# THU-luvision/TextureFusion

Measured on AMD Instinct MI355X. Metric: RGB-D frames/s (TSDF integrate + atlas update: prepare->integrate->finalize, UpdateMeshes, GeneratePatches + UpdateAtlas over the frame's dirty chunks), higher is better.
Workload: dtype f32

## Files before the change

### texturefusion_amd/csrc/tf_mesh.hip

```cpp
#include <stdlib.h>
#include <string.h>

#include <algorithm>
#include <vector>

#include "tf_devfn.h"
#include "tf_kf_store.h"
#include "tf_mc_table.h"
#include "tf_patch_body.h"
#include "tf_volume.h"

#pragma clang fp contract(off)

namespace tf {

__device__ const unsigned long long d_mc_tri[256] = TF_MC_TRI_TABLE_INIT;

constexpr int kR = 11;
constexpr int kRS = 11;
constexpr int kPS = kRS * kR;
constexpr int kRV = kPS * kR;
constexpr int kEdgeSlots = 3 * 729;
__device__ __forceinline__ uint32_t mesh_shard_rows_d(uint32_t max_chunks) { return max_chunks / kMeshShards + 258u; }

// ... 293 lines not shown
template <bool WAVE_FORM, bool PATCH, bool TL = false>
__global__ __launch_bounds__(256, PATCH ? (WAVE_FORM ? TF_FILTER_PATCH_WAVES : TF_FILTER_BATCH_WAVES) : (WAVE_FORM ? TF_FILTER_WAVES : TF_FILTER_BATCH_WAVES)) void k_mesh_filter(VolumeDev v, const int4* __restrict__ dlist,
                                                     const uint32_t* __restrict__ dslot,
                                                     const uint32_t* __restrict__ dcount, uint32_t max_entries,
                                                     uint32_t epoch, uint32_t* __restrict__ surv,
                                                     uint32_t* __restrict__ cnt, uint32_t cap_sh, int ppar, bool use_summ,
                                                     uint32_t* __restrict__ len_hint, int shards_par, FilterPatch fp) {
  if (fp.n_store && blockIdx.x == 0) {
    kf_store_body<256>(v, fp.store.tab, fp.store.slots, fp.store.arena, fp.store.cap, fp.store.slot, fp.store.slack, fp.store.fill);
    return;
  }
  const uint32_t bx = blockIdx.x - fp.n_store, nbx = gridDim.x - fp.n_store;
  if (PATCH && bx - fp.first < fp.n_patch) {
    patch_body<true, true, true>(v, fp.cam, fp.par, fp.kf, bx - fp.first, fp.n_patch);
    return;
  }
  const uint32_t bid = PATCH ? (fp.first ? bx : bx - fp.n_patch) : bx;
  const uint32_t nblk = PATCH ? nbx - fp.n_patch : nbx;
  const int lane = threadIdx.x & 63, w = threadIdx.x >> 6;
  const bool is_near = lane < 27 && (lane % 3) >= 1 && ((lane / 3) % 3) >= 1 && lane / 9 >= 1;
  const uint32_t create_seq = v.vctl->create_seq;
  const uint32_t tl_wave = (bid * 256 + threadIdx.x) >> 6;
  bool tl_first = true;
  auto stamp = [&](int k, bool wait) {
    if (TL && tl_first && tl_wave < (uint32_t)kPhaseWaves) {
      if (wait) asm volatile("s_waitcnt vmcnt(0)" ::: "memory");
      if (lane == 0) v.phase_buf[tl_wave * 16 + k] = __builtin_amdgcn_s_memrealtime();
    }
  };
  if (TL && lane == 0 && tl_wave < (uint32_t)kPhaseWaves) { for (int k = 1; k < 8; ++k) v.phase_buf[tl_wave * 16 + k] = 0; }
  stamp(0, false);
  uint32_t n_flat = *dcount;
  if (n_flat > max_entries) n_flat = max_entries;
  const uint32_t wl_rows = mesh_shard_rows_d(v.max_chunks);
  const size_t wl_base = (size_t)(shards_par & 1) * kMeshShards * wl_rows;
  uint32_t sh_n = 0, sh_incl = 0;
  if (shards_par >= 0 && (!WAVE_FORM || bid == 0)) {
    if (lane < (int)kMeshShards) { sh_n = v.wl_cnt[((shards_par & 1) * kMeshShards + lane) * 16]; if (sh_n > wl_rows) sh_n = wl_rows; }
    sh_incl = sh_n;
#pragma unroll
    for (int o = 1; o < (int)kMeshShards; o <<= 1) {
      const uint32_t u = (uint32_t)__shfl_up((int)sh_incl, o);
      if (lane >= o) sh_incl += u;
    }
  }
  const uint32_t n_sh = (uint32_t)__builtin_amdgcn_readfirstlane(__shfl((int)sh_incl, kMeshShards - 1));
  uint32_t n = n_flat + n_sh;
  if (n > max_entries) n = max_entries;
  if (len_hint && bid == 0 && threadIdx.x == 0) *len_hint = n;
  const uint32_t nwaves = nblk * 4;
  if (WAVE_FORM) {
    const uint32_t wave = (uint32_t)__builtin_amdgcn_readfirstlane((int)((bid * 256 + threadIdx.x) >> 6));
    auto process = [&](const int4 id, const uint32_t own_listed, const bool have_own) {
      if (fp.cls && ((fp.cls == 1u) != part_interior(v, id.x, id.y, id.z))) return;
      const uint32_t own = have_own ? own_listed : hash_slot_alive(v, pack_id(id.x, id.y, id.z));
      if (own == kInvalidSlot) return;
      const bool claimed = have_own && id.w > 0;
      const uint32_t roww = load_here(&v.nbr[(size_t)own * kNbrWords + (lane & (kNbrWords - 1))]);
      const uint32_t alivew = v.hent[claimed ? (uint32_t)id.w - 1u : 0u].alive;
      uint32_t w = lane < kNbrWords ? roww : 0u;
      const uint32_t alive = claimed ? (alivew & 1u) : 1u;
      stamp(2, true);
      if (!alive) return;
      w = nbr_row_checked(v, own, id, lane, w, create_seq);
      const uint32_t nslot = lane == 13 ? own : ((lane < 27 && w) ? w - 1u : kInvalidSlot);
      if (use_summ) {
        const uint32_t sm = (is_near && nslot != kInvalidSlot) ? v.summ[nslot] : 0u;
        const uint32_t sel = lane == 13 ? 0u : ((lane % 3) == 2 ? 4u : (((lane / 3) % 3) == 2 ? 8u : 12u));
        const uint32_t u = is_near ? (sm >> sel) & 15u : 0u;
        const bool so = (__shfl((int)sm, 13) & 1) != 0;
        stamp(3, true);
        const bool maybe = so && __ballot(u & 2u) != 0ull && __ballot(u & 4u) != 0ull && __ballot(u & 8u) != 0ull;
        if (!maybe) {
          if (lane == 0) { if (fp.defer) filter_defer_reset(v, cnt, cap_sh, own, id); else filter_reset_record(v, own, id, epoch, ppar); }
          stamp(4, true);
          return;
        }
      }
      filter_exact<true>(v, id, nslot, own, lane, epoch, surv, cnt, cap_sh, ppar, use_summ, fp.defer != 0, create_seq);
      stamp(5, true);
    };
    if (shards_par >= 0) {
      const uint32_t sd = wave & (kMeshShards - 1u);
      const uint32_t stride = (nwaves - sd + kMeshShards - 1u) / kMeshShards;
      uint32_t i = wave / kMeshShards;
      size_t at = wl_base + (size_t)sd * wl_rows + (i < wl_rows ? i : 0u);
      const unsigned long long* const idq = reinterpret_cast<const unsigned long long*>(&v.wl_ids[at]);
      const unsigned long long id_lo = load_here(idq), id_hi = load_here(idq + 1);
      uint32_t own_listed = load_here(&v.wl_slot[at]);
      uint32_t cs = load_here(&v.wl_cnt[((shards_par & 1) * kMeshShards + sd) * 16]);
      int4 id = make_int4((int)(uint32_t)id_lo, (int)(uint32_t)(id_lo >> 32), (int)(uint32_t)id_hi, (int)(uint32_t)(id_hi >> 32));
      if (cs > wl_rows) cs = wl_rows;
      stamp(1, true);
      while (i < cs) {
        process(id, own_listed, true);
        stamp(6, false);
        tl_first = false;
        i += stride;
        if (i < cs) { at = wl_base + (size_t)sd * wl_rows + i; id = v.wl_ids[at]; own_listed = v.wl_slot[at]; }
      }
    }
    for (uint32_t entry = wave; entry < n_flat; entry += nwaves) {
      const int4 id = dlist[entry];
      uint32_t own_listed = kInvalidSlot;
      if (dslot) own_listed = dslot[entry];
      process(id, own_listed, dslot != nullptr);
    }
    return;
  }
  __shared__ uint32_t s_n, s_ne;
  __shared__ uint32_t s_incl[kMeshShards], s_cnt[kMeshShards];
  if (threadIdx.x < kMeshShards) { s_incl[threadIdx.x] = sh_incl; s_cnt[threadIdx.x] = sh_n; }
  __shared__ uint32_t s_eown[32];
  __shared__ int4 s_eid[32];
  __shared__ int4 s_id[32];
  __shared__ uint32_t s_own[32];
  const int grp = threadIdx.x >> 3, k8 = threadIdx.x & 7;
  const uint32_t per = (n + nblk - 1) / nblk;
  const uint32_t first = bid * per;
  const uint32_t last = first + per < n ? first + per : n;
  for (uint32_t base = first; base < last; base += 32u) {
    if (threadIdx.x == 0) { s_n = 0; s_ne = 0; }
    __syncthreads();
    const uint32_t entry = base + (uint32_t)grp;
    if (entry < last) {
      int4 id;
      uint32_t own_in = kInvalidSlot;
      if (entry < n_flat) {
        id = dlist[entry];
        own_in = dslot ? dslot[entry] : hash_slot_alive(v, pack_id(id.x, id.y, id.z));
      } else {
        const uint32_t r = entry - n_flat;
        uint32_t shd = 0;
        for (uint32_t q = 0; q < kMeshShards; ++q) shd += s_incl[q] <= r ? 1u : 0u;
        shd &= kMeshShards - 1u;
        const size_t at = wl_base + (size_t)shd * wl_rows + (r - (s_incl[shd] - s_cnt[shd]));
        id = v.wl_ids[at];
        own_in = v.wl_slot[at];
      }
      uint32_t own;
      bool maybe;
      filter_near(v, id, lane, k8, own_in, dslot != nullptr || entry >= n_flat, use_summ, create_seq, &own, &maybe);
      if (fp.cls && ((fp.cls == 1u) != part_interior(v, id.x, id.y, id.z))) own = kInvalidSlot;
      if (own != kInvalidSlot && k8 == 0) {
        if (maybe) {
          const uint32_t at = atomicAdd(&s_n, 1u);
          s_own[at] = own; s_id[at] = id;
        } else {
          const uint32_t at = atomicAdd(&s_ne, 1u);
          s_eown[at] = own; s_eid[at] = id;
        }
      }
    }
    __syncthreads();
    if (w == 3 && lane < (int)s_ne) {
      if (fp.defer) filter_defer_reset(v, cnt, cap_sh, s_eown[lane], s_eid[lane]);
      else filter_reset_record(v, s_eown[lane], s_eid[lane], epoch, ppar);
    }
    const uint32_t nm = s_n;
    for (uint32_t m = (uint32_t)w; m < nm; m += 4u)
      filter_exact<false>(v, s_id[m], kInvalidSlot, s_own[m], lane, epoch, surv, cnt, cap_sh, ppar, use_summ, fp.defer != 0, create_seq);
    __syncthreads();
  }
}

__device__ __forceinline__ void mesh_stamp(const VolumeDev& v, uint32_t r, int k) {
  if (threadIdx.x == 0 && blockIdx.x < (uint32_t)kPhaseWaves && r == blockIdx.x)
    v.phase_buf[blockIdx.x * 16 + k] = __builtin_amdgcn_s_memrealtime();
}

#ifndef TF_MESH_WAVES
#define TF_MESH_WAVES 6
#endif
template <int NT, bool DBG = false>
__global__ __launch_bounds__(NT, TF_MESH_WAVES) void k_mesh(VolumeDev v, const uint32_t* __restrict__ surv, uint32_t* __restrict__ cnt,
                                                 uint32_t* __restrict__ cnt_next, uint32_t cap_sh,
                                                 uint32_t epoch, float res, uint32_t simplified, uint32_t dbg,
                                                 int rearm) {
  __shared__ MeshSh<NT> sh;
  extern __shared__ uint16_t vlist[];
  const int t = threadIdx.x, lane = t & 63;
  uint32_t n_rows = 0, excl_l = 0, incl_l = 0;
  {
    uint32_t my_n = cnt[(lane & 31) * 16 + (lane >> 5)];
    if (my_n > cap_sh) my_n = cap_sh;
    uint32_t incl = my_n;
#pragma unroll
    for (int o = 1; o < 64; o <<= 1) {
      const uint32_t u = (uint32_t)__shfl_up((int)incl, o);
      if (lane >= o) incl += u;
    }
    n_rows = (uint32_t)__builtin_amdgcn_readfirstlane(__shfl((int)incl, 63));
    const uint32_t r0 = blockIdx.x;
    const uint32_t sh0 = (uint32_t)__popcll(__ballot(incl <= r0));
    incl_l = (uint32_t)__builtin_amdgcn_readfirstlane(__shfl((int)incl, (int)(sh0 & 63u)));
    excl_l = incl_l - (uint32_t)__builtin_amdgcn_readfirstlane(__shfl((int)my_n, (int)(sh0 & 63u)));
    incl_l = (uint32_t)__builtin_amdgcn_readfirstlane((int)sh0);
  }
  if (blockIdx.x == 0 && t < (int)kMeshShards) { cnt_next[t * 16] = 0u; cnt_next[t * 16 + 1] = 0u; cnt_next[(kMeshShards + t) * 16] = 0u; cnt_next[(kMeshShards + t) * 16 + 1] = 0u; cnt_next[(2 * kMeshShards + t) * 16] = 0u; }
  if (blockIdx.x < kMeshShards) {
    uint32_t n_reset = cnt[(2u * kMeshShards + blockIdx.x) * 16u];
    if (n_reset > cap_sh) n_reset = cap_sh;
    for (uint32_t i = (uint32_t)t; i < n_reset; i += NT) {
      const int4 e = v.reset_list[(size_t)blockIdx.x * cap_sh + i];
      filter_reset_record(v, (uint32_t)e.w, make_int4(e.x, e.y, e.z, 0), epoch, rearm >= 0 ? (rearm ^ 1) : -1);
    }
  }
  const float half = res * 0.5f;
  if (rearm >= 0 && blockIdx.x == 0 && t == 0) {
    AtlasCtl::Set* O = &v.actl->set[rearm];
    O->n_work = 0; O->n_cand = 0; O->n_patch = 0; O->slots_base = 0ull;
    v.actl->set[rearm ^ 1].slots_base = v.actl->n_slots;
  }
  if (rearm >= 0 && blockIdx.x == 0 && t < (int)kMeshShards) {
    v.patch_cnt[((rearm & 1) * kMeshShards + t) * 16] = 0u;
    v.wl_cnt[((rearm & 1) * kMeshShards + t) * 16] = 0u;
  }
  if (DBG && dbg == 9) mesh_stamp(v, blockIdx.x, 0);
  for (uint32_t r = blockIdx.x; r < n_rows; r += gridDim.x) {
    uint32_t shard, own;
    int4 id;
    float2 a[512 / NT];
    unsigned long long htab[(kHalo + NT - 1) / NT];
    uint32_t rstate0, rblock0, rpress0;
    unsigned long long rtexloc0;
    {
      shard = incl_l;
      uint32_t idx = r - excl_l;
      if (r != blockIdx.x) {
        uint32_t my_n = cnt[(lane & 31) * 16 + (lane >> 5)];
        if (my_n > cap_sh) my_n = cap_sh;
        uint32_t incl = my_n;
#pragma unroll
        for (int o = 1; o < 64; o <<= 1) {
          const uint32_t u = (uint32_t)__shfl_up((int)incl, o);
          if (lane >= o) incl += u;
        }
        shard = (uint32_t)__builtin_amdgcn_readfirstlane((int)__popcll(__ballot(incl <= r)));
        idx = r - (uint32_t)__builtin_amdgcn_readfirstlane(__shfl((int)incl, (int)(shard & 63u)) - __shfl((int)my_n, (int)(shard & 63u)));
      }
      if (shard >= kMeshShards) { shard -= kMeshShards; idx = cap_sh - 1u - idx; }
      const size_t row = (size_t)shard * cap_sh + idx;
      own = surv[32 * row + 13];
      id = make_int4((int)surv[32 * row + 27], (int)surv[32 * row + 28], (int)surv[32 * row + 29], 0);
#pragma unroll
      for (int j = 0; j < 512 / NT; ++j) a[j] = v.tsdf[(size_t)own * kChunkVoxels + j * NT + t];
      const uint32_t roww = load_here(&surv[32 * row + (t & 31)]);
      int th = threadIdx.x;
      asm volatile("" : "+v"(th));
#pragma unroll
      for (int j = 0; j < (kHalo + NT - 1) / NT; ++j) {
        const int at = j * NT + th;
        const unsigned long long e = d_mesh_tabs.halo[(j + 1) * NT <= kHalo ? at : (at < kHalo ? at : kHalo - 1)];
        htab[j] = ((j + 1) * NT <= kHalo || at < kHalo) ? e : ~0ull;
      }
      const MeshRec* const rec0 = &v.mesh_rec[own];
      rstate0 = rec0->state; rblock0 = rec0->block; rpress0 = blk_pressure(v); rtexloc0 = rec0->texloc;
      __syncthreads();
      if (t < 27) sh.nslot[t] = roww;
    }
    int t_ = threadIdx.x;
    asm volatile("" : "+v"(t_));
    const int t = t_, lane = t & 63, w = t >> 6;
    MeshRec* rec = &v.mesh_rec[own];
    if (DBG && dbg == 9) mesh_stamp(v, r, 1);
    if (t == 0) { sh.nv = 0; sh.nt = 0; sh.adj = 0; sh.ncell = 0; }
    if (DBG && dbg == 1) continue;
#pragma unroll
    for (int j = 0; j < 512 / NT; ++j) {
      const int q = j * NT + t;
      const int x0 = q & 7, y0 = (q >> 3) & 7, z0 = q >> 6;
      sh.S[ridx(x0, y0, z0)] = a[j].x; sh.cflag[x0 + y0 * 9 + z0 * 81] = (a[j].y > 50.0f) ? kCfHeavy : 0u;
    }
    if (t == NT - 64) { sh.rstate = rstate0; sh.rblock = rblock0; sh.rtexloc = rtexloc0; sh.rpress = rpress0; }
    __syncthreads();
    float4 hv[(kHalo + NT - 1) / NT];
    bool hhave[(kHalo + NT - 1) / NT];
#pragma unroll
    for (int j = 0; j < (kHalo + NT - 1) / NT; ++j) {
      const unsigned long long e = htab[j];
      const uint32_t nb = (uint32_t)(e >> 11) & 31u;
      const uint32_t s = sh.nslot[nb < 26u ? nb : 26u];
      hhave[j] = e != ~0ull && s != kInvalidSlot;
      hv[j] = reinterpret_cast<const float4*>(v.tsdf + (size_t)(hhave[j] ? s : own) * kChunkVoxels)[hhave[j] ? (uint32_t)(e >> 16) & 255u : 0u];
    }
#pragma unroll
    for (int j = 0; j < (kHalo + NT - 1) / NT; ++j) {
      const unsigned long long e = htab[j];
      const float4 val = hhave[j] ? hv[j] : make_float4(999.0f, 0.0f, 999.0f, 0.0f);
      const uint32_t r0 = (uint32_t)e & 2047u;
      if (e != ~0ull && ((e >> 24) & 1ull)) {
        sh.S[r0] = val.x;
        const uint32_t cf = (uint32_t)(e >> 26) & 1023u;
        if (cf) sh.cflag[cf - 1u] = (val.y > 50.0f) ? kCfHeavy : 0u;
      }
      if (e != ~0ull && ((e >> 25) & 1ull)) {
        sh.S[r0 + 1u] = val.z;
        const uint32_t cf = (uint32_t)(e >> 36) & 1023u;
        if (cf) sh.cflag[cf - 1u] = (val.w > 50.0f) ? kCfHeavy : 0u;
      }
    }
    __syncthreads();
    if (DBG && dbg == 9) mesh_stamp(v, r, 3);
    for (int c = t; c < 729; c += NT) {
      const int r = ridx(c % 9, (c / 9) % 9, c / 81);
      const float xm = sh.S[r - 1], xp = sh.S[r + 1], ym = sh.S[r - kRS], yp = sh.S[r + kRS];
      const float zm = sh.S[r - kPS], zp = sh.S[r + kPS];
      uint32_t f = (xm < 1.0f ? 1u : 0u) | (xp < 1.0f ? 2u : 0u) | (ym < 1.0f ? 4u : 0u) | (yp < 1.0f ? 8u : 0u) |
                   (zm < 1.0f ? 16u : 0u) | (zp < 1.0f ? 32u : 0u);
      const float gx = xp - xm, gy = yp - ym, gz = zp - zm;
      const float yz = gy * gy + gz * gz;
      const float nrm = sqrtf(gx * gx + yz);
      if (!(nrm > res * 100.0f)) f |= kCfGradOk;
      sh.cflag[c] |= (uint8_t)f;
    }
    for (int i = t; i < (kEdgeSlots + 7) / 8; i += NT) sh.ownq[i] = 0u;
    __syncthreads();

    if (DBG && dbg == 2) continue;
    if (DBG && dbg == 9) mesh_stamp(v, r, 4);
    for (int cell = t; cell < 512; cell += NT) {
      const int x = cell & 7, y = (cell >> 3) & 7, z = cell >> 6;
      const int c0 = ridx(x, y, z);
      bool observed = true;
      int pos = 0, index = 0;
#pragma unroll
      for (int k = 0; k < 8; ++k) {
        const float s = sh.S[c0 + cox(k) + coy(k) * kRS + coz(k) * kPS];
        observed = observed && !(s > 1.0f);
        pos += (s > 0.0f) ? 1 : 0;
        index |= (0.0f > s) ? (1 << k) : 0;
      }
      sh.cinfo[cell] = 0;
      if (observed && (pos % 8) > 0 && index != 0 && index != 255)
        sh.clist[atomicAdd(&sh.ncell, 1u)] = (uint16_t)cell;
    }
    __syncthreads();
    if (t == 0 && sh.ncell) atomicAdd(&cnt[(kMeshShards + shard) * 16 + 1], 1u);
    for (uint32_t ci = t; ci < sh.ncell; ci += NT) {
      const int cell = sh.clist[ci];
      const int x = cell & 7, y = (cell >> 3) & 7, z = cell >> 6;
      const int c0 = ridx(x, y, z);
      float cube[8];
      int index = 0;
#pragma unroll
      for (int k = 0; k < 8; ++k) {
        const float s = sh.S[c0 + cox(k) + coy(k) * kRS + coz(k) * kPS];
        cube[k] = s;
        index |= (0.0f > s) ? (1 << k) : 0;
      }
      const unsigned long long row = d_mc_tri[index];
      uint32_t valid = 0;
      const int cf0 = x + y * 9 + z * 81;
#pragma unroll
      for (int e = 0; e < 12; ++e) {
        const int e0 = (int)((0x321076543210ull >> (4 * e)) & 0xF), e1 = (int)((0x765447650321ull >> (4 * e)) & 0xF);
        const float s0 = cube[e0], s1 = cube[e1];
        const bool far = fabsf(s0) > fabsf(s1);
        const int ko = far ? (cox(e1) + coy(e1) * 9 + coz(e1) * 81) : (cox(e0) + coy(e0) * 9 + coz(e0) * 81);
        const uint32_t need0 = kCfHeavy | kCfGradOk | (1u << cox(e0)) | (4u << coy(e0)) | (16u << coz(e0));
        const uint32_t need1 = kCfHeavy | kCfGradOk | (1u << cox(e1)) | (4u << coy(e1)) | (16u << coz(e1));
        const uint32_t need = far ? need1 : need0;
        if (s0 * s1 < 0.0f) {
          const uint32_t have = sh.cflag[cf0 + ko];
          if ((have & need) == need) valid |= 1u << e;
        }
      }
      uint32_t ntri = 0, used = 0;
#pragma unroll 1
      for (int col = 0; col < 15; col += 3) {
        const int s0 = (int)((row >> (4 * col)) & 0xF);
        if (s0 == 0xF) break;
        const int s1 = (int)((row >> (4 * col + 4)) & 0xF), s2 = (int)((row >> (4 * col + 8)) & 0xF);
        if (!((valid >> s0) & (valid >> s1) & (valid >> s2) & 1u)) continue;
        ++ntri;
        used |= (1u << s0) | (1u << s1) | (1u << s2);
      }
      for (uint32_t u = used; u; u &= u - 1) {
        const int e = __builtin_ctz(u);
        const int m = edge_slot(x, y, z, e);
        atomicOr(&sh.ownq[m >> 3], 1u << (4 * (m & 7) + edge_q(e)));
      }
      sh.cinfo[cell] = (uint16_t)(used | (ntri << 12));
      sh.cidx[cell] = (uint8_t)index;
    }
    __syncthreads();

    if (DBG && dbg == 3) continue;
    if (DBG && dbg == 9) mesh_stamp(v, r, 5);
    {
      constexpr int kEpt = 2304 / NT, kCpt = 512 / NT;
      const int first = t * kEpt;
      unsigned long long usedm = 0;
      {
        constexpr int kWords = (kEpt * 4 + 31) / 32 + 1;
        const int w0 = first >> 3, sh0 = 4 * (first & 7);
#pragma unroll
        for (int q = 0; q < kWords; ++q) {
          const int wi = w0 + q;
          uint32_t x = wi < (kEdgeSlots + 7) / 8 ? sh.ownq[wi] : 0u;
          x |= x >> 1; x |= x >> 2; x &= 0x11111111u;
          x = (x | (x >> 3)) & 0x03030303u;
          x = (x | (x >> 6)) & 0x000F000Fu;
          x = (x | (x >> 12)) & 0xFFu;
          usedm |= (unsigned long long)x << (8 * q);
        }
        usedm >>= (sh0 >> 2);
        usedm &= (1ull << kEpt) - 1ull;
        const int left = kEdgeSlots - first;
        if (left < kEpt) usedm = left > 0 ? (usedm & ((1ull << left) - 1ull)) : 0ull;
      }
      const uint32_t cnt = (uint32_t)__popcll(usedm);
      uint32_t tc = 0;
#pragma unroll
      for (int j = 0; j < kCpt; ++j) tc += (uint32_t)sh.cinfo[kCpt * t + j] >> 12;
      uint32_t pk = cnt | (tc << 16);
      uint32_t inc = pk;
#pragma unroll
      for (int o = 1; o < 64; o <<= 1) {
        const uint32_t u = __shfl_up(inc, o);
        if (lane >= o) inc += u;
      }
      if (lane == 63) sh.wsum[w] = inc;
      __syncthreads();
      uint32_t before = 0, total = 0;
      for (int k = 0; k < NT / 64; ++k) {
        if (k < w) before += sh.wsum[k];
        total += sh.wsum[k];
      }
      if (t == 0) sh.ovf = mesh_block_for(v, sh.rblock, total & 0xFFFFu, total >> 16, sh.rpress);
      __syncthreads();
      const uint32_t ovf_blk = sh.ovf;
      uint16_t* const gvl = (ovf_blk != kBlkFail && (ovf_blk & kBlkLarge)) ? v.ovf_vlist + (size_t)((ovf_blk & ~kBlkLarge) - 1u) * kOvfCV : nullptr;
      const uint32_t excl = before + inc - pk;
      uint32_t r = excl & 0xFFFFu;
      sh.rbase[t] = (uint16_t)r;
      sh.rmask[t] = usedm;
      for (unsigned long long u = usedm; u; u &= u - 1ull) {
        const int m = first + (int)__builtin_ctzll(u);
        if (gvl) { if (r < (uint32_t)kOvfCV) gvl[r] = (uint16_t)m; }
        else if (r < v.mesh_cv) vlist[r] = (uint16_t)m;
        ++r;
      }
      uint32_t t0 = excl >> 16;
#pragma unroll
      for (int j = 0; j < kCpt; ++j) {
        sh.toff[kCpt * t + j] = (uint16_t)t0;
        t0 += (uint32_t)sh.cinfo[kCpt * t + j] >> 12;
      }
      if (t == 0) { sh.nv = total & 0xFFFFu; sh.nt = total >> 16; }
    }
    __syncthreads();
    const uint32_t nv = sh.nv, nt = sh.nt;
    const uint32_t ovf = sh.ovf;
    if (ovf == kBlkFail) {
      if (t == 0) {
        atomicOr(&v.vctl->status, kStMeshFull);
        const uint32_t was = sh.rstate & kMsInMap;
        rec->nv = 0; rec->nt = 0; rec->state = was | kMsOverflow; rec->epoch = epoch;
        if (rearm >= 0 && was) patch_list_append(v, rearm ^ 1, shard, id, own, sh.rtexloc, sh.rblock);
      }
      __syncthreads();
      continue;
    }
    const uint16_t* const gvlist = (ovf & kBlkLarge) ? v.ovf_vlist + (size_t)((ovf & ~kBlkLarge) - 1u) * kOvfCV : nullptr;

    if (DBG && dbg == 4) continue;
    if (DBG && dbg == 9) mesh_stamp(v, r, 6);
    const uint32_t inmap = (sh.rstate & kMsInMap) | (nv ? kMsInMap : 0u);
    if (t == NT - 64) {
      mesh_block_settle(v, sh.rblock, ovf);
      if (rearm >= 0 && inmap) patch_list_append(v, rearm ^ 1, shard, id, own, sh.rtexloc, ovf);
    }
    const float org[3] = {(float)(8 * id.x) * res, (float)(8 * id.y) * res, (float)(8 * id.z) * res};
    uint32_t adj = 0;
    for (uint32_t i = t; i < nv; i += NT) {
      const int m = gvlist ? gvlist[i] : vlist[i];
      const int cell = owner_cell(m, __builtin_ctz((sh.ownq[m >> 3] >> (4 * (m & 7))) & 0xFu));
      const int x = cell & 7, y = (cell >> 3) & 7, z = cell >> 6;
      const int ax = m % 3, b = m / 3;
      const int bx = b % 9, by = (b / 9) % 9, bz = b / 81;
      const int e = edge_of_slot(ax, bx - x, by - y, bz - z);
      const int e0 = edge_c0(e), e1 = edge_c1(e);
      const float s0 = sh.S[ridx(x + cox(e0), y + coy(e0), z + coz(e0))];
      const float s1 = sh.S[ridx(x + cox(e1), y + coy(e1), z + coz(e1))];
      const float tt = s0 / (s0 - s1);
      const int o0[3] = {cox(e0), coy(e0), coz(e0)}, o1[3] = {cox(e1), coy(e1), coz(e1)};
      const int cc[3] = {x, y, z};
      float pv[3];
#pragma unroll
      for (int a = 0; a < 3; ++a) {
        const float p0 = (float)o0[a] * res, p1 = (float)o1[a] * res;
        const float ev = p0 + tt * (p1 - p0);
        const float origin = org[a] + ((float)cc[a] * res + half);
        pv[a] = ev + origin;
      }
      const int k = (fabsf(s0) > fabsf(s1)) ? e1 : e0;
      const int px = x + cox(k), py = y + coy(k), pz = z + coz(k);
      float g[3];
      gradient_at(sh.S, px, py, pz, cox(k), coy(k), coz(k), res, g);
      const uint32_t cs = sh.nslot[((px + 8) >> 3) + ((py + 8) >> 3) * 3 + ((pz + 8) >> 3) * 9];
      const unsigned long long c4 = load_here(reinterpret_cast<const unsigned long long*>(v.color + (size_t)cs * kChunkVoxels + (px & 7) + (py & 7) * 8 + (pz & 7) * 64));
      float col[3] = {1.0f, 1.0f, 1.0f};
      const float cw = (float)(uint16_t)(c4 >> 48);
      if (cw > 0.0f) {
        col[0] = ((float)(uint16_t)c4 / 255.0f) / cw;
        col[1] = ((float)(uint16_t)(c4 >> 16) / 255.0f) / cw;
        col[2] = ((float)(uint16_t)(c4 >> 32) / 255.0f) / cw;
      }
#pragma unroll
      for (int a = 0; a < 3; ++a) {
        mesh_plane(v, ovf, kMpPos + a)[i] = pv[a];
        mesh_plane(v, ovf, kMpNrm + a)[i] = g[a];
        mesh_plane(v, ovf, kMpCol + a)[i] = col[a];
        const int gp = (int)floorf((pv[a] - org[a]) / (res * 1.0f));
        if (gp >= 8) adj |= 1u << (2 * a + 1);
        if (gp <= 0) adj |= 1u << (2 * a);
      }
    }
    if (adj) atomicOr(&sh.adj, adj);
    if (DBG && dbg == 9) mesh_stamp(v, r, 7);
    for (uint32_t ci = (uint32_t)(NT - 1 - t); ci < sh.ncell; ci += NT) {
      const int cell = sh.clist[ci];
      const uint32_t info = sh.cinfo[cell];
      if (!(info >> 12)) continue;
      const int x = cell & 7, y = (cell >> 3) & 7, z = cell >> 6;
      const unsigned long long row = d_mc_tri[sh.cidx[cell]];
      const uint32_t valid = info & 0xFFFu;
      uint32_t o = sh.toff[cell];
      for (int col = 0; col < 15; col += 3) {
        const int s0 = (int)((row >> (4 * col)) & 0xF);
        if (s0 == 0xF) break;
        const int s1 = (int)((row >> (4 * col + 4)) & 0xF), s2 = (int)((row >> (4 * col + 8)) & 0xF);
        if (!((valid >> s0) & (valid >> s1) & (valid >> s2) & 1u)) continue;
        constexpr int kEptT = 2304 / NT;
        auto ref_of = [&](int m) {
          const int tt = m / kEptT, j = m - tt * kEptT;
          return (uint16_t)(sh.rbase[tt] + (uint32_t)__popcll(sh.rmask[tt] & ((1ull << j) - 1ull)));
        };
        tri_plane(v, ovf, 0)[o] = ref_of(edge_slot(x, y, z, s2));
        tri_plane(v, ovf, 1)[o] = ref_of(edge_slot(x, y, z, s1));
        tri_plane(v, ovf, 2)[o] = ref_of(edge_slot(x, y, z, s0));
        ++o;
      }
    }
    __syncthreads();
    if (t == 0) {
      rec->nv = (uint16_t)nv; rec->nt = (uint16_t)nt; rec->epoch = epoch; rec->block = ovf;
      rec->state = inmap | (sh.adj << kMsAdjShift) | (inmap ? simplified : 0u);
    }
    __syncthreads();
    if (DBG && dbg == 9) mesh_stamp(v, r, 8);
  }
}

__global__ __launch_bounds__(256) void k_init_mesh_rec(MeshRec* rec, uint32_t n) {
  for (uint32_t i = blockIdx.x * 256 + threadIdx.x; i < n; i += gridDim.x * 256) {
    MeshRec r;
    memset(&r, 0, sizeof(r));
    r.texloc = kNoTexloc;
    r.frameid = -1;
    r.ratio[0] = r.ratio[1] = 1.0f;
    rec[i] = r;
  }
}
void launch_init_meshes(const VolumeDev& v, hipStream_t s) {
  hipLaunchKernelGGL(k_init_mesh_rec, dim3(1024), dim3(256), 0, s, v.mesh_rec, v.max_chunks);
  (void)hipMemsetAsync(v.mesh_rec + v.max_chunks, 0, sizeof(uint32_t) * ((size_t)blk_ring_len(v.mesh_blocks) + blk_ring_len(v.ovf_blocks)), s);
  (void)hipMemsetAsync(v.mesh_cnt, 0, sizeof(uint32_t) * 2 * kMeshCntWords, s);
}

uint32_t mesh_shard_rows(uint32_t max_chunks) { return max_chunks / kMeshShards + 258u; }

static void launch_mesher(const VolumeDev& v, int cnt_par, uint32_t max_entries, uint32_t epoch, float res, bool fused,
                          int rearm_set, hipStream_t s) {
  static const uint32_t dbg = getenv("TF_MESH_DBG") ? (uint32_t)atoi(getenv("TF_MESH_DBG")) : 0u;
  uint32_t* surv = v.mesh_nbr;
  uint32_t* cnt = v.mesh_cnt + (size_t)(cnt_par & 1) * kMeshCntWords;
  uint32_t* cnt_next = v.mesh_cnt + (size_t)((cnt_par & 1) ^ 1) * kMeshCntWords;
  const uint32_t cap_sh = mesh_shard_rows(v.max_chunks);
  uint32_t grid = ((max_entries + kMeshShards - 1) / kMeshShards + 1) * kMeshShards;
  static const uint32_t gmax = (uint32_t)device_cus() * (uint32_t)(TF_MESH_WAVES * 2);
  if (grid > gmax) grid = gmax;
  if (dbg)
    hipLaunchKernelGGL((k_mesh<128, true>), dim3(grid), dim3(128), v.mesh_cv * sizeof(uint16_t), s, v, surv, cnt, cnt_next, cap_sh, epoch, res,
                       fused ? kMsSimplified : 0u, dbg, rearm_set);
  else
    hipLaunchKernelGGL((k_mesh<128>), dim3(grid), dim3(128), v.mesh_cv * sizeof(uint16_t), s, v, surv, cnt, cnt_next, cap_sh, epoch, res,
                       fused ? kMsSimplified : 0u, 0u, rearm_set);
}

bool launch_mesh(const VolumeDev& v, int cnt_par, const int4* dlist, const uint32_t* dcount, uint32_t max_entries,
                 uint32_t epoch, float res, bool fused, int rearm_set, uint32_t len_guess, uint32_t* len_hint, int shards_par,
                 hipStream_t s, const PatchStage* patch, const Cam* cam, int cls, const KfStoreArgs* store) {
  if (!max_entries) return false;
  uint32_t* cnt = v.mesh_cnt + (size_t)(cnt_par & 1) * kMeshCntWords;
  const uint32_t cap_sh = mesh_shard_rows(v.max_chunks);
  if (max_entries > v.max_chunks) max_entries = v.max_chunks;
  const uint32_t fmax = 2560u;
  const uint32_t fgrid = (max_entries + 3) / 4 < fmax ? (max_entries + 3) / 4 : fmax;
  const uint32_t* dslot = fused ? v.work_slot : nullptr;
  const int ppar = fused ? (rearm_set ^ 1) : -1;
  const bool use_summ = true;
  const bool wave_form = len_guess <= 2560u * 4u;
  FilterPatch fp;
  memset(&fp, 0, sizeof(fp));
  fp.cls = (uint32_t)cls;
  if (store) { fp.n_store = 1u; fp.store = *store; }
  if (patch && cam) {
    fp.defer = 1u;
    fp.n_patch = 1024u;
    fp.first = 0u;
    fp.par = patch->par;
    fp.cam = *cam;
    fp.kf = patch->kf;
  }
#define TF_LAUNCH_FILTER(W, P)                                                                                       \
  hipLaunchKernelGGL((k_mesh_filter<W, P>), dim3(fgrid + fp.n_patch + fp.n_store), dim3(256), 0, s, v, dlist, dslot, dcount, max_entries, \
                     epoch, v.mesh_nbr, cnt, cap_sh, ppar, use_summ, len_hint, shards_par, fp)
  static const bool tl = getenv("TF_MESH_DBG") && atoi(getenv("TF_MESH_DBG")) == 10;
  if (wave_form && tl && !fp.n_patch)
    hipLaunchKernelGGL((k_mesh_filter<true, false, true>), dim3(fgrid + fp.n_store), dim3(256), 0, s, v, dlist, dslot, dcount, max_entries,
                       epoch, v.mesh_nbr, cnt, cap_sh, ppar, use_summ, len_hint, shards_par, fp);
  else if (wave_form) { if (fp.n_patch) TF_LAUNCH_FILTER(true, true); else TF_LAUNCH_FILTER(true, false); }
  else { if (fp.n_patch) TF_LAUNCH_FILTER(false, true); else TF_LAUNCH_FILTER(false, false); }
#undef TF_LAUNCH_FILTER
  launch_mesher(v, cnt_par, max_entries, epoch, res, fused, rearm_set, s);
  return fp.n_patch != 0;
}

constexpr uint32_t kDirtyBlocks = 512;
__device__ __forceinline__ void dirty_frame_body(const VolumeDev& v, int par, uint32_t stamp) {
  const SelBuf& L = v.sel;
  const uint32_t nl = L.ctl->n_list <= v.max_list ? L.ctl->n_list : 0u;
  const uint32_t total = nl * 8u;
  AtlasCtl::Set* S = &v.actl->set[par];
  const int lane = threadIdx.x & 63, w = threadIdx.x >> 6;
  __shared__ uint32_t wcnt[16];
  __shared__ uint32_t gbase;
  for (uint32_t b0 = blockIdx.x * 1024; b0 < total; b0 += kDirtyBlocks * 1024) {
    const uint32_t t = b0 + threadIdx.x;
    bool emit = false;
    int4 q = make_int4(0, 0, 0, 0);
    uint32_t slot = kInvalidSlot;
    if (t < total && (t & 7u) != 7u) {
      const uint32_t e = list_phys(v, t >> 3, L.ctl->n_front);
      const int k = (int)(t & 7u);
      const int4 id0 = L.list_id[e];
      const uint32_t slot0 = L.list_slot[e];
      if (L.list_needs[e]) {
        q = nbr7(id0, k);
        q.w = 0;
        if (k == 0) slot = slot0;
        else slot = hash_slot_alive(v, pack_id(q.x, q.y, q.z));
        if (slot != kInvalidSlot && part_owned(v, q.x, q.y, q.z))
          emit = atomicMax(&v.mesh_rec[slot].stamp, stamp) < stamp;
      }
    }
    const unsigned long long m = __ballot(emit);
    if (lane == 0) wcnt[w] = (uint32_t)__popcll(m);
    __syncthreads();
    if (threadIdx.x == 0) {
      uint32_t tot = 0;
      for (int k = 0; k < 16; ++k) { const uint32_t c = wcnt[k]; wcnt[k] = tot; tot += c; }
      gbase = tot ? atomicAdd(&S->n_work, tot) : 0u;
    }
    __syncthreads();
    if (emit) {
      const uint32_t p = gbase + wcnt[w] + (uint32_t)__popcll(m & ((1ull << lane) - 1ull));
// ... 438 lines not shown
```

Before: 11070.

## Fuse corner-flag pass into cell classification and compute flags lazily per active cell

Drops the separate pass that computed neighbour-observed and gradient-ok flags for all 729 corners. Those flags are now computed on demand only for the corners of surface-crossing cells. Cell classification is restructured so each thread walks a z-column and reuses the previous z-plane's four samples, which roughly halves the shared-memory reads, and one __syncthreads is removed. The trade-off is redundant flag work for corners shared by several active cells, plus more register pressure and divergence inside the active-cell loop.

New measurement: 11140, median of 3. Within noise of the previous version (+0.6%).

```diff
diff --git a/texturefusion_amd/csrc/tf_mesh.hip b/texturefusion_amd/csrc/tf_mesh.hip
--- a/texturefusion_amd/csrc/tf_mesh.hip
+++ b/texturefusion_amd/csrc/tf_mesh.hip
@@ -619,40 +619,37 @@
     }
     __syncthreads();
     if (DBG && dbg == 9) mesh_stamp(v, r, 3);
-    for (int c = t; c < 729; c += NT) {
-      const int r = ridx(c % 9, (c / 9) % 9, c / 81);
-      const float xm = sh.S[r - 1], xp = sh.S[r + 1], ym = sh.S[r - kRS], yp = sh.S[r + kRS];
-      const float zm = sh.S[r - kPS], zp = sh.S[r + kPS];
-      uint32_t f = (xm < 1.0f ? 1u : 0u) | (xp < 1.0f ? 2u : 0u) | (ym < 1.0f ? 4u : 0u) | (yp < 1.0f ? 8u : 0u) |
-                   (zm < 1.0f ? 16u : 0u) | (zp < 1.0f ? 32u : 0u);
-      const float gx = xp - xm, gy = yp - ym, gz = zp - zm;
-      const float yz = gy * gy + gz * gz;
-      const float nrm = sqrtf(gx * gx + yz);
-      if (!(nrm > res * 100.0f)) f |= kCfGradOk;
-      sh.cflag[c] |= (uint8_t)f;
+    if (DBG && dbg == 2) continue;
+    {
+      constexpr int kZr = 512 / NT;
+      const int x = t & 7, y = (t >> 3) & 7, z0 = (t >> 6) * kZr;
+      const int c0 = ridx(x, y, z0);
+      bool obs_lo = true;
+      int pos_lo = 0, neg_lo = 0;
+#pragma unroll
+      for (int l = 0; l <= kZr; ++l) {
+        bool obs = true;
+        int pos = 0, neg = 0;
+#pragma unroll
+        for (int k = 0; k < 4; ++k) {
+          const float s = sh.S[c0 + cox(k) + coy(k) * kRS + l * kPS];
+          obs = obs && !(s > 1.0f);
+          pos += (s > 0.0f) ? 1 : 0;
+          neg |= (0.0f > s) ? (1 << k) : 0;
+        }
+        if (l > 0) {
+          const int cell = x + 8 * y + 64 * (z0 + l - 1);
+          const int index = neg_lo | (neg << 4);
+          sh.cinfo[cell] = 0;
+          if (obs_lo && obs && ((pos_lo + pos) % 8) > 0 && index != 0 && index != 255)
+            sh.clist[atomicAdd(&sh.ncell, 1u)] = (uint16_t)cell;
+        }
+        obs_lo = obs; pos_lo = pos; neg_lo = neg;
+      }
     }
     for (int i = t; i < (kEdgeSlots + 7) / 8; i += NT) sh.ownq[i] = 0u;
     __syncthreads();
-
-    if (DBG && dbg == 2) continue;
     if (DBG && dbg == 9) mesh_stamp(v, r, 4);
-    for (int cell = t; cell < 512; cell += NT) {
-      const int x = cell & 7, y = (cell >> 3) & 7, z = cell >> 6;
-      const int c0 = ridx(x, y, z);
-      bool observed = true;
-      int pos = 0, index = 0;
-#pragma unroll
-      for (int k = 0; k < 8; ++k) {
-        const float s = sh.S[c0 + cox(k) + coy(k) * kRS + coz(k) * kPS];
-        observed = observed && !(s > 1.0f);
-        pos += (s > 0.0f) ? 1 : 0;
-        index |= (0.0f > s) ? (1 << k) : 0;
-      }
-      sh.cinfo[cell] = 0;
-      if (observed && (pos % 8) > 0 && index != 0 && index != 255)
-        sh.clist[atomicAdd(&sh.ncell, 1u)] = (uint16_t)cell;
-    }
-    __syncthreads();
     if (t == 0 && sh.ncell) atomicAdd(&cnt[(kMeshShards + shard) * 16 + 1], 1u);
     for (uint32_t ci = t; ci < sh.ncell; ci += NT) {
       const int cell = sh.clist[ci];
@@ -667,21 +664,33 @@
         index |= (0.0f > s) ? (1 << k) : 0;
       }
       const unsigned long long row = d_mc_tri[index];
+      const int cf0 = x + y * 9 + z * 81;
+      bool cok[8];
+#pragma unroll
+      for (int k = 0; k < 8; ++k) {
+        const int ox = cox(k), oy = coy(k), oz = coz(k);
+        const int rk = c0 + ox + oy * kRS + oz * kPS;
+        const float xo = sh.S[rk + (ox ? 1 : -1)], yo = sh.S[rk + (oy ? kRS : -kRS)], zo = sh.S[rk + (oz ? kPS : -kPS)];
+        const float xi = cube[4 * oz + (oy ? 2 + ox : 1 - ox)], yi = cube[4 * oz + (oy ? ox : 3 - ox)], zi = cube[k ^ 4];
+        const float xm = ox ? xi : xo, xp = ox ? xo : xi;
+        const float ym = oy ? yi : yo, yp = oy ? yo : yi;
+        const float zm = oz ? zi : zo, zp = oz ? zo : zi;
+        uint32_t have = sh.cflag[cf0 + ox + oy * 9 + oz * 81];
+        have |= (xo < 1.0f ? (1u << ox) : 0u) | (yo < 1.0f ? (4u << oy) : 0u) | (zo < 1.0f ? (16u << oz) : 0u);
+        const float gx = xp - xm, gy = yp - ym, gz = zp - zm;
+        const float yz = gy * gy + gz * gz;
+        const float nrm = sqrtf(gx * gx + yz);
+        if (!(nrm > res * 100.0f)) have |= kCfGradOk;
+        const uint32_t need = kCfHeavy | kCfGradOk | (1u << ox) | (4u << oy) | (16u << oz);
+        cok[k] = (have & need) == need;
+      }
       uint32_t valid = 0;
-      const int cf0 = x + y * 9 + z * 81;
 #pragma unroll
       for (int e = 0; e < 12; ++e) {
         const int e0 = (int)((0x321076543210ull >> (4 * e)) & 0xF), e1 = (int)((0x765447650321ull >> (4 * e)) & 0xF);
         const float s0 = cube[e0], s1 = cube[e1];
         const bool far = fabsf(s0) > fabsf(s1);
-        const int ko = far ? (cox(e1) + coy(e1) * 9 + coz(e1) * 81) : (cox(e0) + coy(e0) * 9 + coz(e0) * 81);
-        const uint32_t need0 = kCfHeavy | kCfGradOk | (1u << cox(e0)) | (4u << coy(e0)) | (16u << coz(e0));
-        const uint32_t need1 = kCfHeavy | kCfGradOk | (1u << cox(e1)) | (4u << coy(e1)) | (16u << coz(e1));
-        const uint32_t need = far ? need1 : need0;
-        if (s0 * s1 < 0.0f) {
-          const uint32_t have = sh.cflag[cf0 + ko];
-          if ((have & need) == need) valid |= 1u << e;
-        }
+        if (s0 * s1 < 0.0f && (far ? cok[e1] : cok[e0])) valid |= 1u << e;
       }
       uint32_t ntri = 0, used = 0;
 #pragma unroll 1
```
